# eragonruan/text-detection-ctpn

Hardware: NVIDIA H100
Metric: images/sec @600x900 (higher is better)
Workload: dtype fp32-faithful: fp16 operands + e4m3 cross terms (1 fp16 + 1 e4m3 wgmma per 16 MACs: 2 bf16-rate units per MAC), fp32 accumulate; matmuls around the BiLSTM on bf16x2

## Files before the change

### text-detection-ctpn_b200/csrc/conv_tc.cu

```cuda
#include <cuda.h>

#include <algorithm>
#include <mutex>
#include <unordered_map>

#include "common.cuh"
#include "tc_ptx.cuh"
#include "tma_host.cuh"

namespace ctpn {

#ifdef CTPN_DEBUG
#define CTPN_DBG(p, bit) (((p).debug & (bit)) != 0)
#else
#define CTPN_DBG(p, bit) false
#endif

struct ConvTcParams {
  int B, H, W, Cin, Cout, taps, planes, flags;
  int tiles_x, tiles_y, tiles_n, total_tiles;
  int m_tiles, total_units;
  int TH, TW, tw_log2;
  int PW;
  int patch_bytes;
  int patch_tx_bytes;
  int group_stride_bytes;
  int cout_pad;
  int Ho, Wo;
  int stages_a, stages_b;
  int debug;
  const float *bias;
  void *out;
  long long out_plane_stride;
  float inv_main, inv_cross, out_s, out_t, out_rs;
  int in_stack_h, out_rows, out_stacked;
  const int *ext;
  int ext_shift, ext_n;
  double work;
  int stage_small;
  int promote_every;
};

constexpr int kTcThreads = 384;
constexpr int kMaxStages = 8;
constexpr int kCtrlBytes = 8 * (4 * kMaxStages) + 16;
constexpr int kStagePitch = 64;
constexpr int kEpiBytes = 2 * 128 * 32 * 4;

template <int BN, int P, int TAPS, int MC, int F8, int PR = 0>
__global__ void __launch_bounds__(kTcThreads, 1)
conv_tc_kernel(const __grid_constant__ CUtensorMap tmap_a, const __grid_constant__ CUtensorMap tmap_b,
               const ConvTcParams p) {
  using namespace ptx;
  constexpr int kBBytes = BN * 128;
  static_assert(!F8 || P == 2, "F16F8 uses two stage slots per operand");
  static_assert(!PR || (P == 3 && !F8), "promotion is built for three bf16 planes");
  extern __shared__ uint8_t smem_raw[];
  const uint32_t raw = smem_u32(smem_raw);
  const uint32_t ring_a = (raw + 1023u) & ~1023u;
  const uint32_t a_stage = (uint32_t)P * p.patch_bytes, b_stage = (uint32_t)P * kBBytes;
  const uint32_t ring_b = ring_a + (uint32_t)p.stages_a * a_stage;
  float *epi = reinterpret_cast<float *>(smem_raw + (ring_b - raw) + (size_t)p.stages_b * b_stage);
  uint8_t *ctrl = reinterpret_cast<uint8_t *>(epi) + kEpiBytes;
  const uint32_t fullA = smem_u32(ctrl), emptyA = fullA + 8 * kMaxStages;
  const uint32_t fullB = emptyA + 8 * kMaxStages, emptyB = fullB + 8 * kMaxStages;

  const int warp = __shfl_sync(0xffffffffu, (int)(threadIdx.x >> 5), 0), lane = threadIdx.x & 31;
  if (threadIdx.x == 0) {
    prefetch_tmap(&tmap_a);
    prefetch_tmap(&tmap_b);
    for (int s = 0; s < kMaxStages; ++s) {
      mbar_init(fullA + 8 * s, 1);
      mbar_init(emptyA + 8 * s, 2);
      mbar_init(fullB + 8 * s, 1);
      mbar_init(emptyB + 8 * s, MC ? 4 : 2);
    }
    fence_mbar_init();
  }
  __syncthreads();
  if (MC) cluster_sync_all();
  const uint32_t rank = MC ? cluster_ctarank() : 0u;
  const int u_begin = MC ? (int)(blockIdx.x >> 1) : (int)blockIdx.x, u_step = MC ? (int)(gridDim.x >> 1) : (int)gridDim.x;
  auto unit_tile = [&](int u, int &mt, int &nt) {
    nt = u % p.tiles_n;
    mt = u / p.tiles_n;
    if (MC) mt = min(2 * mt + (int)rank, p.m_tiles - 1);
  };

  const int kblocks = p.Cin / 64;
  const int tiles_per_img = p.tiles_x * p.tiles_y;
  constexpr int halo = TAPS == 9 ? 1 : 0;

  if (warp < 4) {
    regs_dealloc<40>();
    if (warp == 1) {
      int s = 0;
      uint32_t ph = 0;
      for (int u = u_begin; u < p.total_units; u += u_step) {
        int mt, nt;
        unit_tile(u, mt, nt);
        const int b = mt / tiles_per_img, r = mt % tiles_per_img;
        const int y0 = (r / p.tiles_x) * p.TH - halo, x0 = (r % p.tiles_x) * p.TW - halo;
        for (int kb = 0; kb < kblocks; ++kb) {
          mbar_wait(emptyA + 8 * s, ph ^ 1u);
          if (elect_one()) {
            if (CTPN_DBG(p, 2)) { mbar_arrive(fullA + 8 * s); }
            else {
              mbar_arrive_expect_tx(fullA + 8 * s, (uint32_t)P * (uint32_t)p.patch_tx_bytes);
              for (int pl = 0; pl < P; ++pl)
                tma_load_4d(&tmap_a, fullA + 8 * s, ring_a + s * a_stage + pl * p.patch_bytes, kb * 64, x0, y0, pl * p.B + b);
            }
          }
          __syncwarp();
          if (++s == p.stages_a) { s = 0; ph ^= 1u; }
        }
      }
    } else if (warp == 0) {
      int s = 0;
      uint32_t ph = 0;
      for (int u = u_begin; u < p.total_units; u += u_step) {
        int mt, nt;
        unit_tile(u, mt, nt);
        for (int kb = 0; kb < kblocks; ++kb) {
          for (int tap = 0; tap < TAPS; ++tap) {
            mbar_wait(emptyB + 8 * s, ph ^ 1u);
            if (elect_one()) {
              if (CTPN_DBG(p, 1)) { mbar_arrive(fullB + 8 * s); }
              else {
                mbar_arrive_expect_tx(fullB + 8 * s, b_stage);
                for (int pl = 0; pl < P; ++pl) {
                  if (MC)
                    tma_load_2d_mc(&tmap_b, fullB + 8 * s, ring_b + s * b_stage + pl * kBBytes + rank * (kBBytes / 2),
                                   tap * p.Cin + kb * 64, pl * p.cout_pad + nt * BN + (int)rank * (BN / 2), (uint16_t)3);
                  else
                    tma_load_2d(&tmap_b, fullB + 8 * s, ring_b + s * b_stage + pl * kBBytes, tap * p.Cin + kb * 64,
                                pl * p.cout_pad + nt * BN);
                }
              }
            }
            __syncwarp();
            if (++s == p.stages_b) { s = 0; ph ^= 1u; }
          }
        }
      }
    }
  } else {
    regs_alloc<232>();
    const int wg = (warp >> 2) - 1;
    const bool leader = (threadIdx.x & 127) == 0;
    constexpr int R = BN / 2;
    float accm[R], accc[R];
    float accs[R];
#ifdef CTPN_DEBUG
    const int pe = PR ? p.promote_every : 1;
#else
    constexpr int pe = 1;
#endif
    constexpr uint32_t kPatch16 = (TAPS == 9 ? 23552u : 16384u) >> 4;
    constexpr uint32_t kB16 = (uint32_t)kBBytes >> 4;
    constexpr uint32_t kHiB = gmma_desc_hi(1024);
    const uint32_t hi_a = gmma_desc_hi((uint32_t)p.group_stride_bytes);
    const uint32_t wg_off = (uint32_t)wg * 8u * (uint32_t)p.group_stride_bytes;
    const int cw = warp - 4, eset = cw >> 2, quarter = cw & 3;
    const int m = quarter * 32 + lane;
    const int th = m >> p.tw_log2, tw = m & (p.TW - 1);
    const bool pool = (p.flags & CTPN_F_POOL) != 0, relu = (p.flags & CTPN_F_RELU) != 0;
    const bool out_f32 = (p.flags & CTPN_F_OUT_F32) != 0;
    int sa = 0, sb = 0, prev_b = -1, prev_a = -1;
    uint32_t pha = 0, phb = 0;
    auto release = [&](int sbx, int sax) {
      if (leader) {
        if (MC) {
          mbar_arrive_cluster(emptyB + 8 * sbx, 0u);
          mbar_arrive_cluster(emptyB + 8 * sbx, 1u);
        } else {
          mbar_arrive(emptyB + 8 * sbx);
        }
        if (sax >= 0) mbar_arrive(emptyA + 8 * sax);
      }
    };
    for (int u = u_begin; u < p.total_units; u += u_step) {
      if (PR) {
#pragma unroll
        for (int i = 0; i < R; ++i) accs[i] = 0.f;
      }
      for (int kb = 0; kb < kblocks; ++kb) {
        if (p.stages_a == 1 && prev_a >= 0) {
          wgmma_wait<0>();
          release(prev_b, prev_a);
          prev_b = prev_a = -1;
        }
        mbar_wait(fullA + 8 * sa, pha);
        const uint32_t a_lo = gmma_desc_lo(ring_a + sa * a_stage + wg_off);
#pragma unroll
        for (int tap = 0; tap < TAPS; ++tap) {
          mbar_wait(fullB + 8 * sb, phb);
          const uint32_t b_lo = gmma_desc_lo(ring_b + sb * b_stage);
          constexpr int kPW = 10;
          const uint32_t view16 = TAPS == 9 ? (uint32_t)((tap / 3) * kPW + tap % 3) * 8u : 0u;
          const uint32_t not_first = (kb | tap) != 0;
          const int step = kb * TAPS + tap;
          wgmma_fence();
          if (!CTPN_DBG(p, 4)) {
            if (F8) {
#pragma unroll
              for (int k = 0; k < 4; ++k)
                wgmma_f16(accm, ((uint64_t)hi_a << 32) | (a_lo + view16 + 2u * k), ((uint64_t)kHiB << 32) | (b_lo + 2u * k),
                          k == 0 ? not_first : 1u);
#pragma unroll
              for (int k = 0; k < 4; ++k)
                wgmma_e4m3(accc, ((uint64_t)hi_a << 32) | (a_lo + kPatch16 + view16 + 2u * k),
                           ((uint64_t)kHiB << 32) | (b_lo + kB16 + 2u * k), k == 0 ? not_first : 1u);
            } else if (PR) {
              const uint32_t chain_on = step % pe != 0;
#pragma unroll
              for (int k = 0; k < 4; ++k)
                wgmma_bf16(accm, ((uint64_t)hi_a << 32) | (a_lo + view16 + 2u * k), ((uint64_t)kHiB << 32) | (b_lo + 2u * k),
                           k == 0 ? chain_on : 1u);
              wgmma_commit();
#pragma unroll
              for (int i = 0; i < P; ++i) {
#pragma unroll
                for (int j = (i == 0); j < P - i; ++j) {
#pragma unroll
                  for (int k = 0; k < 4; ++k) {
                    const uint64_t da = ((uint64_t)hi_a << 32) | (a_lo + i * kPatch16 + view16 + 2u * k);
                    const uint64_t db = ((uint64_t)kHiB << 32) | (b_lo + j * kB16 + 2u * k);
                    wgmma_bf16(accc, da, db, (k == 0 && i == 0 && j == 1) ? not_first : 1u);
                  }
                }
              }
            } else {
#pragma unroll
              for (int i = 0; i < P; ++i) {
#pragma unroll
                for (int j = 0; j < P - i; ++j) {
#pragma unroll
                  for (int k = 0; k < 4; ++k) {
                    const uint64_t da = ((uint64_t)hi_a << 32) | (a_lo + i * kPatch16 + view16 + 2u * k);
                    const uint64_t db = ((uint64_t)kHiB << 32) | (b_lo + j * kB16 + 2u * k);
                    if (i + j == 0) wgmma_bf16(accm, da, db, k == 0 ? not_first : 1u);
                    else wgmma_bf16(accc, da, db, (k == 0 && i == 0 && j == 1) ? not_first : 1u);
                  }
                }
              }
            }
          }
          wgmma_commit();
          wgmma_wait<1>();
          if (prev_b >= 0) release(prev_b, prev_a);
          prev_b = sb;
          prev_a = tap == TAPS - 1 ? sa : -1;
          if (PR && ((step + 1) % pe == 0 || step == kblocks * TAPS - 1)) {
            wgmma_fence_regs(accm);
#pragma unroll
            for (int i = 0; i < R; ++i) accs[i] = __fadd_rn(accs[i], accm[i]);
          }
          if (++sb == p.stages_b) { sb = 0; phb ^= 1u; }
        }
        if (++sa == p.stages_a) { sa = 0; pha ^= 1u; }
      }
      wgmma_wait<0>();
      wgmma_fence_regs(accm);
      if (P > 1) wgmma_fence_regs(accc);
      if (prev_b >= 0) release(prev_b, prev_a);
      prev_b = prev_a = -1;
      if (P > 1) {
#pragma unroll
        for (int i = 0; i < R; ++i)
          accm[i] = F8 ? __fmaf_rn(accc[i], p.inv_cross, accm[i] * p.inv_main) : PR ? __fadd_rn(accs[i], accc[i]) : accm[i] + accc[i];
      }

      int mt, nt;
      unit_tile(u, mt, nt);
      const int b = mt / tiles_per_img, r = mt % tiles_per_img;
      const int y = (r / p.tiles_x) * p.TH + th, x = (r % p.tiles_x) * p.TW + tw;
      bool ok, live = true;
      int oy, ox, ob = b;
      if (pool) {
        oy = y >> 1; ox = x >> 1;
        ok = !(th & 1) && !(tw & 1) && oy < p.Ho && ox < p.Wo;
      } else {
        oy = y; ox = x;
        ok = y < p.H && x < p.W;
        if (p.in_stack_h) {
          ob = y / p.in_stack_h;
          oy = y - ob * p.in_stack_h;
          live = oy < p.in_stack_h - 1;
          if (!p.out_stacked) ok = ok && live;
        }
      }
      if (p.ext) {
        const int ib = min(ob, p.ext_n - 1);
        live = live && oy < (__ldg(p.ext + 2 * ib) >> p.ext_shift) && ox < (__ldg(p.ext + 2 * ib + 1) >> p.ext_shift);
      }
      const long long pix = ((long long)ob * p.out_rows + oy) * p.Wo + ox;
      const unsigned okmask = __ballot_sync(0xffffffffu, ok);
      long long spix[4];
#pragma unroll
      for (int it = 0; it < 4; ++it) {
        const long long hi = __shfl_sync(0xffffffffu, (int)(pix >> 32), it * 8 + (lane >> 2));
        const unsigned lo = __shfl_sync(0xffffffffu, (unsigned)(pix & 0xffffffffll), it * 8 + (lane >> 2));
        spix[it] = (hi << 32) | lo;
      }
      uint4 *stage_w = reinterpret_cast<uint4 *>(epi + eset * 4096 + quarter * 1024);
      const int frow = wg * 64 + (warp & 3) * 16 + (lane >> 2);
      if (!CTPN_DBG(p, 16)) {
#pragma unroll
      for (int c2 = 0; c2 < BN / 64; ++c2) {
        named_sync(1, 256);
#pragma unroll
        for (int j = 0; j < 8; ++j) {
          const int i8 = c2 * 8 + j, q = 2 * (j & 3) + ((lane & 3) >> 1);
#pragma unroll
          for (int h = 0; h < 2; ++h) {
            const int row = frow + 8 * h;
            *reinterpret_cast<float2 *>(epi + (j >> 2) * 4096 + row * 32 + ((q ^ (row & 7)) << 2) + 2 * (lane & 1)) =
                make_float2(accm[4 * i8 + 2 * h], accm[4 * i8 + 2 * h + 1]);
          }
        }
        named_sync(1, 256);
        const int chunk = 2 * c2 + eset;
        const int c0 = nt * BN + chunk * 32;
        float v[32];
#pragma unroll
        for (int q = 0; q < 8; ++q) {
          const float4 t = *reinterpret_cast<const float4 *>(epi + eset * 4096 + m * 32 + ((q ^ (m & 7)) << 2));
          v[4 * q + 0] = t.x; v[4 * q + 1] = t.y; v[4 * q + 2] = t.z; v[4 * q + 3] = t.w;
        }
#pragma unroll
        for (int q = 0; q < 8; ++q) {
          const float4 bq = __ldg(reinterpret_cast<const float4 *>(p.bias + c0) + q);
          v[4 * q + 0] += bq.x;
          v[4 * q + 1] += bq.y;
          v[4 * q + 2] += bq.z;
          v[4 * q + 3] += bq.w;
        }
        if (relu) {
#pragma unroll
          for (int i = 0; i < 32; ++i) v[i] = fmaxf(v[i], 0.f);
        }
        if (!live) {
#pragma unroll
          for (int i = 0; i < 32; ++i) v[i] = 0.f;
        }
        if (pool) {
#pragma unroll
          for (int i = 0; i < 32; ++i) {
            v[i] = fmaxf(v[i], __shfl_xor_sync(0xffffffffu, v[i], 1));
            v[i] = fmaxf(v[i], __shfl_xor_sync(0xffffffffu, v[i], p.TW));
          }
        }
        if (F8 && pool && !out_f32 && !(p.flags & CTPN_F_OUT_BF16X2)) {
          const int j = (lane & 1) | ((lane >> 2) & 2);
          float x[8];
#pragma unroll
          for (int k = 0; k < 8; ++k) x[k] = j == 0 ? v[k] : j == 1 ? v[8 + k] : j == 2 ? v[16 + k] : v[24 + k];
          const bool okw = oy < p.Ho && ox < p.Wo;
          uint4 hw;
          uint2 qv, qr;
          f16f8_quad(x[0], x[1], x[2], x[3], p.out_s, p.out_t, p.out_rs, hw.x, hw.y, qv.x, qr.x);
          f16f8_quad(x[4], x[5], x[6], x[7], p.out_s, p.out_t, p.out_rs, hw.z, hw.w, qv.y, qr.y);
          if (okw && c0 < p.Cout && !CTPN_DBG(p, 8)) {
            uint8_t *o0 = reinterpret_cast<uint8_t *>(p.out) + pix * p.Cout * 2;
            uint8_t *o1 = o0 + p.out_plane_stride * 2 + (long long)(c0 >> 6) * 128 + (c0 & 63) + j * 8;
            *reinterpret_cast<uint4 *>(o0 + (long long)c0 * 2 + j * 16) = hw;
            *reinterpret_cast<uint2 *>(o1) = qv;
            *reinterpret_cast<uint2 *>(o1 + 64) = qr;
          }
        } else if (F8 && !out_f32 && !(p.flags & CTPN_F_OUT_BF16X2)) {
          uint32_t wh[16], wq[16];
#pragma unroll
          for (int i = 0; i < 8; ++i) {
            f16f8_quad(v[4 * i], v[4 * i + 1], v[4 * i + 2], v[4 * i + 3], p.out_s, p.out_t, p.out_rs, wh[2 * i], wh[2 * i + 1], wq[i], wq[8 + i]);
          }
          const int j = lane & 3;
#pragma unroll
          for (int pl = 0; pl < 2; ++pl) {
            uint8_t *obase = reinterpret_cast<uint8_t *>(p.out) + (long long)pl * p.out_plane_stride * 2;
            const long long off = pl == 0 ? (long long)c0 * 2 + j * 16
                                          : (long long)(c0 >> 6) * 128 + (c0 & 63) + (j >> 1) * 64 + (j & 1) * 16;
            const bool st_ok = c0 < p.Cout && !CTPN_DBG(p, 8);
            if (!p.stage_small) {
              __syncwarp();
#pragma unroll
              for (int q = 0; q < 4; ++q) {
                const uint4 val = pl == 0 ? make_uint4(wh[4 * q], wh[4 * q + 1], wh[4 * q + 2], wh[4 * q + 3])
                                          : make_uint4(wq[4 * q], wq[4 * q + 1], wq[4 * q + 2], wq[4 * q + 3]);
                stage_w[lane * 4 + (q ^ ((lane >> 1) & 3))] = val;
              }
              __syncwarp();
              if (st_ok) {
#pragma unroll
                for (int it = 0; it < 4; ++it) {
                  const int pp = it * 8 + (lane >> 2);
                  const uint4 val = stage_w[pp * 4 + (j ^ ((pp >> 1) & 3))];
                  if ((okmask >> pp) & 1u) *reinterpret_cast<uint4 *>(obase + spix[it] * p.Cout * 2 + off) = val;
                }
              }
            } else {
#pragma unroll
              for (int it = 0; it < 4; ++it) {
                __syncwarp();
                if ((lane >> 3) == it) {
                  const int row = lane & 7;
#pragma unroll
                  for (int q = 0; q < 4; ++q) {
                    const uint4 val = pl == 0 ? make_uint4(wh[4 * q], wh[4 * q + 1], wh[4 * q + 2], wh[4 * q + 3])
                                              : make_uint4(wq[4 * q], wq[4 * q + 1], wq[4 * q + 2], wq[4 * q + 3]);
                    stage_w[row * 4 + (q ^ ((row >> 1) & 3))] = val;
                  }
                }
                __syncwarp();
                const int row = lane >> 2, pp = it * 8 + row;
                const uint4 val = stage_w[row * 4 + (j ^ ((row >> 1) & 3))];
                if (st_ok && ((okmask >> pp) & 1u)) *reinterpret_cast<uint4 *>(obase + spix[it] * p.Cout * 2 + off) = val;
              }
            }
          }
        } else if (!out_f32) {
          uint32_t w[P][16];
#pragma unroll
          for (int i = 0; i < 16; ++i) {
            uint32_t t[P];
            split_planes2<P>(v[2 * i], v[2 * i + 1], t);
#pragma unroll
            for (int pl = 0; pl < P; ++pl) w[pl][i] = t[pl];
          }
#pragma unroll
          for (int pl = 0; pl < P; ++pl) {
            __syncwarp();
#pragma unroll
            for (int q = 0; q < 4; ++q) stage_w[lane * 4 + (q ^ ((lane >> 1) & 3))] = make_uint4(w[pl][4 * q], w[pl][4 * q + 1], w[pl][4 * q + 2], w[pl][4 * q + 3]);
            __syncwarp();
            if (c0 < p.Cout && !CTPN_DBG(p, 8)) {
              __nv_bfloat16 *obase = reinterpret_cast<__nv_bfloat16 *>(p.out) + (long long)pl * p.out_plane_stride + c0 + (lane & 3) * 8;
#pragma unroll
              for (int it = 0; it < 4; ++it) {
                const int pp = it * 8 + (lane >> 2);
                const uint4 val = stage_w[pp * 4 + ((lane & 3) ^ ((pp >> 1) & 3))];
                if ((okmask >> pp) & 1u) *reinterpret_cast<uint4 *>(obase + spix[it] * p.Cout) = val;
              }
            }
          }
        } else if (ok && c0 < p.Cout && !CTPN_DBG(p, 8)) {
          if (out_f32) {
            float4 *dst = reinterpret_cast<float4 *>(reinterpret_cast<float *>(p.out) + pix * p.Cout + c0);
#pragma unroll
            for (int q = 0; q < 8; ++q) dst[q] = make_float4(v[4 * q], v[4 * q + 1], v[4 * q + 2], v[4 * q + 3]);
          }
        }
      }
      }
    }
  }
  __syncthreads();
  if (MC) cluster_sync_all();
}


constexpr int kMaxDevices = 64;
static std::mutex g_mu;
static int g_sms[kMaxDevices];

struct Tuning { int debug = 0, bn = 0, stages_a = 0, stages_b = 0, mcast = 1, stage_small = 1, promote = 1; };
static const Tuning &tuning() {
  static const Tuning t = [] {
    Tuning v;
#ifdef CTPN_DEBUG
    auto env_int = [](const char *name, int dflt) { const char *e = getenv(name); return e ? atoi(e) : dflt; };
    v.debug = env_int("CTPN_TC_DEBUG", 0);
    v.bn = env_int("CTPN_TC_BN", 0);
    v.stages_a = env_int("CTPN_TC_STAGES_A", 0);
    v.stages_b = env_int("CTPN_TC_STAGES_B", 0);
    v.mcast = env_int("CTPN_TC_MCAST", 1);
    v.stage_small = env_int("CTPN_TC_STAGE_SMALL", 1);
    v.promote = std::max(1, env_int("CTPN_TC_PROMOTE", 1));
#endif
    return v;
  }();
  return t;
}

struct TmapKey {
  const void *ptr;
  unsigned long long d0, d1, d2, d3;
  unsigned b0, b1, b2, b3;
  int dev;
  bool operator==(const TmapKey &o) const {
    return ptr == o.ptr && d0 == o.d0 && d1 == o.d1 && d2 == o.d2 && d3 == o.d3 && b0 == o.b0 && b1 == o.b1 && b2 == o.b2 &&
           b3 == o.b3 && dev == o.dev;
  }
};
struct TmapKeyHash {
  size_t operator()(const TmapKey &k) const {
    size_t h = std::hash<const void *>()(k.ptr);
    for (unsigned long long v : {k.d0, k.d1, k.d2, k.d3, (unsigned long long)k.b0, (unsigned long long)k.b1,
                                 (unsigned long long)k.b2, (unsigned long long)k.b3, (unsigned long long)k.dev})
      h = h * 1000003u ^ std::hash<unsigned long long>()(v);
    return h;
  }
};
static std::unordered_map<TmapKey, CUtensorMap, TmapKeyHash> g_tmaps;

static int cached_tmap(int dev, CUtensorMap *out, const void *ptr, int rank, const cuuint64_t *dims, const cuuint64_t *strides,
                       const cuuint32_t *box) {
  TmapKey k{ptr, dims[0], dims[1], rank > 2 ? dims[2] : 0, rank > 3 ? dims[3] : 0, box[0], box[1], rank > 2 ? box[2] : 0,
            rank > 3 ? box[3] : 0, dev};
  std::lock_guard<std::mutex> lock(g_mu);
  auto it = g_tmaps.find(k);
  if (it != g_tmaps.end()) { *out = it->second; return CTPN_OK; }
  EncodeTiledFn enc = nullptr;
  int rc = tma_get_encode(&enc);
  if (rc) return rc;
  if ((rc = tma_encode_bf16(enc, out, const_cast<void *>(ptr), rank, dims, strides, box))) return rc;
  if (g_tmaps.size() >= 1024) g_tmaps.clear();
  g_tmaps.emplace(k, *out);
  return CTPN_OK;
}

template <int BN, int P, int TAPS, int MC, int F8 = 0, int PR = 0>
static int launch_bn(int dev, const CUtensorMap &ta, const CUtensorMap &tb, ConvTcParams &p, cudaStream_t st) {
  const size_t a_stage = (size_t)p.planes * p.patch_bytes, b_stage = (size_t)p.planes * BN * 128;
  const bool small = F8 && TAPS == 9 && p.Cin >= 256 && !(p.flags & (CTPN_F_OUT_F32 | CTPN_F_OUT_BF16X2 | CTPN_F_POOL)) && tuning().stage_small != 0;
  p.stage_small = small ? 1 : 0;
  const size_t budget = 227 * 1024 - 1024 - kCtrlBytes - kEpiBytes;
  int sa = (2 * a_stage + 2 * b_stage <= budget) ? 2 : 1;
  if (p.taps == 1) sa = (int)std::min<size_t>(4, std::max<size_t>(1, (budget / 2) / a_stage));
  CTPN_REQUIRE(sa * a_stage + 2 * b_stage <= budget, "conv_tc: pipeline stages (%zu + 2 x %zu B) do not fit in shared memory", a_stage, b_stage);
  int sb = (int)((budget - sa * a_stage) / b_stage);
  if (sb > kMaxStages) sb = kMaxStages;
  if (tuning().stages_a > 0) sa = std::max(1, std::min(sa, tuning().stages_a));
  if (tuning().stages_b > 0) sb = std::max(2, std::min(sb, tuning().stages_b));
  p.stages_a = sa;
  p.stages_b = sb;
  const size_t smem = 1024 + sa * a_stage + sb * b_stage + kEpiBytes + kCtrlBytes;
  CTPN_REQUIRE(smem <= 227 * 1024, "conv_tc: %zu bytes of shared memory", smem);
  auto kernel = conv_tc_kernel<BN, P, TAPS, MC, F8, PR>;
  static bool attr_set[kMaxDevices];
  static int max_clusters[kMaxDevices];
  cudaLaunchConfig_t cfg = {};
  cudaLaunchAttribute attr;
  attr.id = cudaLaunchAttributeClusterDimension;
  attr.val.clusterDim.x = 2; attr.val.clusterDim.y = 1; attr.val.clusterDim.z = 1;
  cfg.blockDim = dim3(kTcThreads);
  cfg.dynamicSmemBytes = smem;
  cfg.stream = st;
  cfg.attrs = &attr;
  cfg.numAttrs = MC ? 1 : 0;
  {
    std::lock_guard<std::mutex> lock(g_mu);
    if (!attr_set[dev]) {
      CTPN_CUDA(cudaFuncSetAttribute(kernel, cudaFuncAttributeMaxDynamicSharedMemorySize, 227 * 1024));
      if (MC) {
        cfg.gridDim = dim3(2 * (g_sms[dev] / 2));
        int n = 0;
        CTPN_CUDA(cudaOccupancyMaxActiveClusters(&n, kernel, &cfg));
        CTPN_REQUIRE(n > 0, "conv_tc: no 2-CTA cluster of this kernel fits on the device");
        max_clusters[dev] = n;
      }
      attr_set[dev] = true;
    }
  }
  char label[128];
  if (prof_enabled()) snprintf(label, sizeof(label), "conv_tc t%d %dx%dx%d c%d-%d %s%d bn%d%s%s", p.taps, p.B, p.H, p.W, p.Cin, p.Cout, F8 ? "f16f8 p" : "p", p.planes, BN, MC ? " mc" : "", PR ? " promote" : "");
  ProfScope prof(label, p.work, st);
  if (MC) cfg.gridDim = dim3(2 * std::min(max_clusters[dev], p.total_units));
  else cfg.gridDim = dim3(std::min(p.total_units, g_sms[dev]));
  CTPN_CUDA(cudaLaunchKernelEx(&cfg, kernel, ta, tb, p));
  CTPN_LAUNCH_CHECK();
  return CTPN_OK;
}

int conv_tc_run(const void *in_planes, const void *w_planes, const float *bias, void *out, int B, int H, int W, int cin,
                int cout, int taps, int planes, int flags, const QuantScales *q, const int *ext, int ext_shift, void *stream) {
  const bool f8 = q != nullptr, promote = (flags & CTPN_F_PROMOTE) != 0;
  CTPN_REQUIRE(f8 || !(flags & CTPN_F_OUT_BF16X2), "ctpn_conv3x3: CTPN_F_OUT_BF16X2 is a flag of ctpn_conv3x3_f16f8");
  CTPN_REQUIRE(!(promote && f8), "ctpn_conv3x3_f16f8: CTPN_F_PROMOTE is a flag of ctpn_conv3x3 with planes = 3");
  CTPN_REQUIRE(!promote || planes == 3, "ctpn_conv3x3: CTPN_F_PROMOTE needs planes = 3 (got %d)", planes);
  CTPN_REQUIRE(in_planes && w_planes && bias && out, "ctpn_conv3x3: null pointer");
  CTPN_REQUIRE(taps == 9 || taps == 1, "ctpn_conv3x3: taps must be 9 or 1 (got %d)", taps);
  CTPN_REQUIRE(planes >= 1 && planes <= 3, "ctpn_conv3x3: planes must be 1..3 (got %d)", planes);
  CTPN_REQUIRE(cin % 64 == 0 && cin >= 64, "ctpn_conv3x3: Cin must be a multiple of 64 (got %d)", cin);
  CTPN_REQUIRE(cout % 64 == 0 && cout >= 64, "ctpn_conv3x3: Cout must be a multiple of 64 (got %d)", cout);
  CTPN_REQUIRE(B > 0 && H > 0 && W > 0, "ctpn_conv3x3: bad shape");
  const bool pool = flags & CTPN_F_POOL;
  CTPN_REQUIRE(!pool || (taps == 9 && H >= 2 && W >= 2), "ctpn_conv3x3: pooling needs taps=9 and H,W >= 2");
  const bool stack_in = flags & CTPN_F_STACK_IN, stack_out = flags & CTPN_F_STACK_OUT;
  CTPN_REQUIRE(!stack_in || (taps == 9 && !pool), "ctpn_conv3x3: CTPN_F_STACK_IN needs taps=9 and no pooling");
  CTPN_REQUIRE(!stack_out || !(flags & CTPN_F_OUT_F32), "ctpn_conv3x3: stacked output is a plane format");
  const int img_B = B, img_H = H;
  if (stack_in) {
    CTPN_REQUIRE((long long)B * (H + 1) < (1ll << 30), "ctpn_conv3x3: stack too tall");
    H = B * (H + 1);
    B = 1;
  }
  int dev = 0, rc;
  CTPN_CUDA(cudaGetDevice(&dev));
  CTPN_REQUIRE(dev >= 0 && dev < kMaxDevices, "ctpn_conv3x3: device index %d not supported", dev);
  {
    std::lock_guard<std::mutex> lock(g_mu);
    if (g_sms[dev] == 0) CTPN_CUDA(cudaDeviceGetAttribute(&g_sms[dev], cudaDevAttrMultiProcessorCount, dev));
  }

  ConvTcParams p;
  memset(&p, 0, sizeof(p));
  p.B = B; p.H = H; p.W = W; p.Cin = cin; p.Cout = cout; p.taps = taps; p.planes = planes; p.flags = flags;
  if (taps == 9) {
    p.TH = 16; p.TW = 8; p.tw_log2 = 3;
    p.PW = 10;
    p.group_stride_bytes = p.PW * 128;
    p.patch_tx_bytes = p.PW * 18 * 128;
    p.patch_bytes = (int)align_up((size_t)p.patch_tx_bytes, 1024);
  } else {
    p.TH = 1; p.TW = 128; p.tw_log2 = 7;
    p.PW = 128;
    p.group_stride_bytes = 1024;
    p.patch_tx_bytes = 128 * 128;
    p.patch_bytes = 128 * 128;
  }
  p.tiles_x = ceil_div(W, p.TW);
  p.tiles_y = ceil_div(H, p.TH);
  p.Ho = pool ? H / 2 : H;
  p.Wo = pool ? W / 2 : W;
  p.bias = bias;
  p.out = out;
  p.work = 2.0 * img_B * img_H * W * (double)taps * cin * cout;
  p.in_stack_h = stack_in ? img_H + 1 : 0;
  const int img_Ho = pool ? img_H / 2 : img_H;
  p.out_rows = img_Ho + (stack_out ? 1 : 0);
  p.out_stacked = stack_out ? 1 : 0;
  p.out_plane_stride = (long long)img_B * p.out_rows * p.Wo * cout;
  p.cout_pad = cout;
  p.ext = ext;
  p.ext_shift = ext_shift;
  p.ext_n = img_B;
  if (f8) {
    CTPN_REQUIRE(q->inv_main > 0.f && q->inv_cross > 0.f && q->out_s > 0.f && q->out_t > 0.f, "ctpn_conv3x3_f16f8: scales must be positive");
    p.inv_main = q->inv_main; p.inv_cross = q->inv_cross; p.out_s = q->out_s; p.out_t = q->out_t;
    p.out_rs = kResidualGain * q->out_t / q->out_s;
  }
  p.debug = tuning().debug;
  p.promote_every = tuning().promote;

  int BN = tuning().bn > 0 ? tuning().bn : (planes == 1 ? 256 : 128);
  if (!(BN == 64 || BN == 128 || BN == 256)) BN = 256;
  if (planes > 1 && BN > 128) BN = 128;
  while (BN > cout || cout % BN) BN >>= 1;
  const long long m_tiles = (long long)B * p.tiles_x * p.tiles_y;
  constexpr long long kMcMaxTilesPerSm = 16;
  const bool mc = taps == 9 && tuning().mcast != 0 && m_tiles >= 2 &&
                  (promote || m_tiles * (cout / BN) < kMcMaxTilesPerSm * g_sms[dev]);
  if (promote && taps == 9 && !mc && BN > 64) BN = 64;
  p.tiles_n = cout / BN;
  const long long total = m_tiles * p.tiles_n;
  CTPN_REQUIRE(total < (1ll << 31), "ctpn_conv3x3: too many tiles");
  p.total_tiles = (int)total;
  p.m_tiles = (int)m_tiles;
  p.total_units = mc ? (int)((m_tiles + 1) / 2) * p.tiles_n : p.total_tiles;

  CUtensorMap ta, tb;
  {
    const int halo = taps == 9 ? 1 : 0;
    cuuint64_t dims[4] = {(cuuint64_t)cin, (cuuint64_t)W, (cuuint64_t)H, (cuuint64_t)planes * B};
    cuuint64_t strides[3] = {(cuuint64_t)cin * 2, (cuuint64_t)W * cin * 2, (cuuint64_t)H * W * cin * 2};
    cuuint32_t box[4] = {64, (cuuint32_t)p.PW, (cuuint32_t)(p.TH + 2 * halo), 1};
    if ((rc = cached_tmap(dev, &ta, in_planes, 4, dims, strides, box))) return rc;
  }
  {
    cuuint64_t dims[2] = {(cuuint64_t)taps * cin, (cuuint64_t)planes * cout};
    cuuint64_t strides[1] = {(cuuint64_t)taps * cin * 2};
    cuuint32_t box[2] = {64, (cuuint32_t)(mc ? BN / 2 : BN)};
    if ((rc = cached_tmap(dev, &tb, w_planes, 2, dims, strides, box))) return rc;
  }
  cudaStream_t st = (cudaStream_t)stream;
#define CTPN_TC_CASE(BN_, P_, T_) \
  if (BN == BN_ && planes == P_ && taps == T_) return launch_bn<BN_, P_, T_, 0>(dev, ta, tb, p, st)
#define CTPN_TC_CASE_MC(BN_, P_) \
  if (mc && BN == BN_ && planes == P_) return launch_bn<BN_, P_, 9, 1>(dev, ta, tb, p, st)
  if (f8) {
    if (mc && BN == 128) return launch_bn<128, 2, 9, 1, 1>(dev, ta, tb, p, st);
    if (mc && BN == 64) return launch_bn<64, 2, 9, 1, 1>(dev, ta, tb, p, st);
    if (taps == 9 && BN == 128) return launch_bn<128, 2, 9, 0, 1>(dev, ta, tb, p, st);
    if (taps == 9 && BN == 64) return launch_bn<64, 2, 9, 0, 1>(dev, ta, tb, p, st);
    if (taps == 1 && BN == 128) return launch_bn<128, 2, 1, 0, 1>(dev, ta, tb, p, st);
    if (taps == 1 && BN == 64) return launch_bn<64, 2, 1, 0, 1>(dev, ta, tb, p, st);
    set_error("ctpn_conv3x3_f16f8: no kernel for BN=%d taps=%d", BN, taps);
    return CTPN_ERR_INVALID;
  }
  if (promote) {
    if (mc && BN == 128) return launch_bn<128, 3, 9, 1, 0, 1>(dev, ta, tb, p, st);
    if (mc && BN == 64) return launch_bn<64, 3, 9, 1, 0, 1>(dev, ta, tb, p, st);
    if (taps == 9 && BN == 64) return launch_bn<64, 3, 9, 0, 0, 1>(dev, ta, tb, p, st);
    if (taps == 1 && BN == 128) return launch_bn<128, 3, 1, 0, 0, 1>(dev, ta, tb, p, st);
    if (taps == 1 && BN == 64) return launch_bn<64, 3, 1, 0, 0, 1>(dev, ta, tb, p, st);
    set_error("ctpn_conv3x3: no promoted kernel for BN=%d taps=%d", BN, taps);
    return CTPN_ERR_INVALID;
  }
  CTPN_TC_CASE_MC(256, 1); CTPN_TC_CASE_MC(128, 1); CTPN_TC_CASE_MC(64, 1);
  CTPN_TC_CASE_MC(128, 2); CTPN_TC_CASE_MC(64, 2);
  CTPN_TC_CASE_MC(128, 3); CTPN_TC_CASE_MC(64, 3);
  CTPN_TC_CASE(256, 1, 9); CTPN_TC_CASE(128, 1, 9); CTPN_TC_CASE(64, 1, 9);
  CTPN_TC_CASE(128, 2, 9); CTPN_TC_CASE(64, 2, 9);
  CTPN_TC_CASE(128, 3, 9); CTPN_TC_CASE(64, 3, 9);
  CTPN_TC_CASE(256, 1, 1); CTPN_TC_CASE(128, 1, 1); CTPN_TC_CASE(64, 1, 1);
  CTPN_TC_CASE(128, 2, 1); CTPN_TC_CASE(64, 2, 1);
  CTPN_TC_CASE(128, 3, 1); CTPN_TC_CASE(64, 3, 1);
#undef CTPN_TC_CASE_MC
#undef CTPN_TC_CASE
  set_error("ctpn_conv3x3: no kernel for BN=%d planes=%d taps=%d", BN, planes, taps);
  return CTPN_ERR_INVALID;
}

}

using namespace ctpn;

extern "C" int ctpn_conv3x3(const void *in_planes, const void *w_planes, const float *bias, void *out, int B, int H,
                            int W, int cin, int cout, int taps, int planes, int flags, void *stream) {
  return conv_tc_run(in_planes, w_planes, bias, out, B, H, W, cin, cout, taps, planes, flags, nullptr, nullptr, 0, stream);
}

extern "C" int ctpn_conv3x3_f16f8(const void *in_planes, const void *w_planes, const float *bias, void *out, int B, int H,
                                  int W, int cin, int cout, int taps, int flags, float inv_main, float inv_cross, float out_s,
                                  float out_t, void *stream) {
  const QuantScales q{inv_main, inv_cross, out_s, out_t};
  return conv_tc_run(in_planes, w_planes, bias, out, B, H, W, cin, cout, taps, 2, flags, &q, nullptr, 0, stream);
}
```

Measured before the change: 762.7.

## Offload conv epilogue to idle producer warps to overlap with next tile's MMA

Adds an epilogue-warp variant where warps 2-3 of the producer group take over bias, ReLU, pooling, quantisation and stores. The consumer warpgroups only dump accumulators to shared memory and then move on to the next tile's wgmma. For wide tiles, chunks beyond the two in the epilogue buffer are staged in the last A pipeline slot, whose release is deferred until the epilogue warps finish. This drops the register dealloc/alloc split, so the MMA warpgroups no longer get the larger 232-register allocation. It also adds mbarrier hand-off latency and can stall the producer on the A slot.

```diff
diff --git a/text-detection-ctpn_b200/csrc/conv_tc.cu b/text-detection-ctpn_b200/csrc/conv_tc.cu
--- a/text-detection-ctpn_b200/csrc/conv_tc.cu
+++ b/text-detection-ctpn_b200/csrc/conv_tc.cu
@@ -46,8 +46,200 @@
 constexpr int kCtrlBytes = 8 * (4 * kMaxStages) + 16;
 constexpr int kStagePitch = 64;
 constexpr int kEpiBytes = 2 * 128 * 32 * 4;
-
-template <int BN, int P, int TAPS, int MC, int F8, int PR = 0>
+constexpr int kChunkFloats = 128 * 32;
+
+__device__ __forceinline__ float *stage_at(float *chunk, int row, int i8, int lane) {
+  const int q = 2 * (i8 & 3) + ((lane & 3) >> 1);
+  return chunk + row * 32 + ((q ^ (row & 7)) << 2) + 2 * (lane & 1);
+}
+
+struct EpiPixel {
+  long long pix;
+  long long spix[4];
+  unsigned okmask;
+  int oy, ox;
+  bool ok, live;
+};
+
+__device__ __forceinline__ EpiPixel epi_pixel(const ConvTcParams &p, int mt, int m, int lane) {
+  EpiPixel e;
+  const int tiles_per_img = p.tiles_x * p.tiles_y;
+  const int th = m >> p.tw_log2, tw = m & (p.TW - 1);
+  const int b = mt / tiles_per_img, r = mt % tiles_per_img;
+  const int y = (r / p.tiles_x) * p.TH + th, x = (r % p.tiles_x) * p.TW + tw;
+  int ob = b;
+  e.live = true;
+  if (p.flags & CTPN_F_POOL) {
+    e.oy = y >> 1; e.ox = x >> 1;
+    e.ok = !(th & 1) && !(tw & 1) && e.oy < p.Ho && e.ox < p.Wo;
+  } else {
+    e.oy = y; e.ox = x;
+    e.ok = y < p.H && x < p.W;
+    if (p.in_stack_h) {
+      ob = y / p.in_stack_h;
+      e.oy = y - ob * p.in_stack_h;
+      e.live = e.oy < p.in_stack_h - 1;
+      if (!p.out_stacked) e.ok = e.ok && e.live;
+    }
+  }
+  if (p.ext) {
+    const int ib = min(ob, p.ext_n - 1);
+    e.live = e.live && e.oy < (__ldg(p.ext + 2 * ib) >> p.ext_shift) && e.ox < (__ldg(p.ext + 2 * ib + 1) >> p.ext_shift);
+  }
+  e.pix = ((long long)ob * p.out_rows + e.oy) * p.Wo + e.ox;
+  e.okmask = __ballot_sync(0xffffffffu, e.ok);
+#pragma unroll
+  for (int it = 0; it < 4; ++it) {
+    const long long hi = __shfl_sync(0xffffffffu, (int)(e.pix >> 32), it * 8 + (lane >> 2));
+    const unsigned lo = __shfl_sync(0xffffffffu, (unsigned)(e.pix & 0xffffffffll), it * 8 + (lane >> 2));
+    e.spix[it] = (hi << 32) | lo;
+  }
+  return e;
+}
+
+template <int P, int F8>
+__device__ __forceinline__ void epi_chunk(const ConvTcParams &p, float *chunk, int m, int lane, int c0, const EpiPixel &e) {
+  const bool pool = (p.flags & CTPN_F_POOL) != 0, relu = (p.flags & CTPN_F_RELU) != 0;
+  const bool out_f32 = (p.flags & CTPN_F_OUT_F32) != 0;
+  const long long pix = e.pix;
+  const int oy = e.oy, ox = e.ox;
+  uint4 *stage_w = reinterpret_cast<uint4 *>(chunk + (m & ~31) * 32);
+  float v[32];
+#pragma unroll
+  for (int q = 0; q < 8; ++q) {
+    const float4 t = *reinterpret_cast<const float4 *>(chunk + m * 32 + ((q ^ (m & 7)) << 2));
+    v[4 * q + 0] = t.x; v[4 * q + 1] = t.y; v[4 * q + 2] = t.z; v[4 * q + 3] = t.w;
+  }
+#pragma unroll
+  for (int q = 0; q < 8; ++q) {
+    const float4 bq = __ldg(reinterpret_cast<const float4 *>(p.bias + c0) + q);
+    v[4 * q + 0] += bq.x;
+    v[4 * q + 1] += bq.y;
+    v[4 * q + 2] += bq.z;
+    v[4 * q + 3] += bq.w;
+  }
+  if (relu) {
+#pragma unroll
+    for (int i = 0; i < 32; ++i) v[i] = fmaxf(v[i], 0.f);
+  }
+  if (!e.live) {
+#pragma unroll
+    for (int i = 0; i < 32; ++i) v[i] = 0.f;
+  }
+  if (pool) {
+#pragma unroll
+    for (int i = 0; i < 32; ++i) {
+      v[i] = fmaxf(v[i], __shfl_xor_sync(0xffffffffu, v[i], 1));
+      v[i] = fmaxf(v[i], __shfl_xor_sync(0xffffffffu, v[i], p.TW));
+    }
+  }
+  if (F8 && pool && !out_f32 && !(p.flags & CTPN_F_OUT_BF16X2)) {
+    const int j = (lane & 1) | ((lane >> 2) & 2);
+    float x[8];
+#pragma unroll
+    for (int k = 0; k < 8; ++k) x[k] = j == 0 ? v[k] : j == 1 ? v[8 + k] : j == 2 ? v[16 + k] : v[24 + k];
+    const bool okw = oy < p.Ho && ox < p.Wo;
+    uint4 hw;
+    uint2 qv, qr;
+    f16f8_quad(x[0], x[1], x[2], x[3], p.out_s, p.out_t, p.out_rs, hw.x, hw.y, qv.x, qr.x);
+    f16f8_quad(x[4], x[5], x[6], x[7], p.out_s, p.out_t, p.out_rs, hw.z, hw.w, qv.y, qr.y);
+    if (okw && c0 < p.Cout && !CTPN_DBG(p, 8)) {
+      uint8_t *o0 = reinterpret_cast<uint8_t *>(p.out) + pix * p.Cout * 2;
+      uint8_t *o1 = o0 + p.out_plane_stride * 2 + (long long)(c0 >> 6) * 128 + (c0 & 63) + j * 8;
+      *reinterpret_cast<uint4 *>(o0 + (long long)c0 * 2 + j * 16) = hw;
+      *reinterpret_cast<uint2 *>(o1) = qv;
+      *reinterpret_cast<uint2 *>(o1 + 64) = qr;
+    }
+  } else if (F8 && !out_f32 && !(p.flags & CTPN_F_OUT_BF16X2)) {
+    uint32_t wh[16], wq[16];
+#pragma unroll
+    for (int i = 0; i < 8; ++i) {
+      f16f8_quad(v[4 * i], v[4 * i + 1], v[4 * i + 2], v[4 * i + 3], p.out_s, p.out_t, p.out_rs, wh[2 * i], wh[2 * i + 1], wq[i], wq[8 + i]);
+    }
+    const int j = lane & 3;
+#pragma unroll
+    for (int pl = 0; pl < 2; ++pl) {
+      uint8_t *obase = reinterpret_cast<uint8_t *>(p.out) + (long long)pl * p.out_plane_stride * 2;
+      const long long off = pl == 0 ? (long long)c0 * 2 + j * 16
+                                    : (long long)(c0 >> 6) * 128 + (c0 & 63) + (j >> 1) * 64 + (j & 1) * 16;
+      const bool st_ok = c0 < p.Cout && !CTPN_DBG(p, 8);
+      if (!p.stage_small) {
+        __syncwarp();
+#pragma unroll
+        for (int q = 0; q < 4; ++q) {
+          const uint4 val = pl == 0 ? make_uint4(wh[4 * q], wh[4 * q + 1], wh[4 * q + 2], wh[4 * q + 3])
+                                    : make_uint4(wq[4 * q], wq[4 * q + 1], wq[4 * q + 2], wq[4 * q + 3]);
+          stage_w[lane * 4 + (q ^ ((lane >> 1) & 3))] = val;
+        }
+        __syncwarp();
+        if (st_ok) {
+#pragma unroll
+          for (int it = 0; it < 4; ++it) {
+            const int pp = it * 8 + (lane >> 2);
+            const uint4 val = stage_w[pp * 4 + (j ^ ((pp >> 1) & 3))];
+            if ((e.okmask >> pp) & 1u) *reinterpret_cast<uint4 *>(obase + e.spix[it] * p.Cout * 2 + off) = val;
+          }
+        }
+      } else {
+#pragma unroll
+        for (int it = 0; it < 4; ++it) {
+          __syncwarp();
+          if ((lane >> 3) == it) {
+            const int row = lane & 7;
+#pragma unroll
+            for (int q = 0; q < 4; ++q) {
+              const uint4 val = pl == 0 ? make_uint4(wh[4 * q], wh[4 * q + 1], wh[4 * q + 2], wh[4 * q + 3])
+                                        : make_uint4(wq[4 * q], wq[4 * q + 1], wq[4 * q + 2], wq[4 * q + 3]);
+              stage_w[row * 4 + (q ^ ((row >> 1) & 3))] = val;
+            }
+          }
+          __syncwarp();
+          const int row = lane >> 2, pp = it * 8 + row;
+          const uint4 val = stage_w[row * 4 + (j ^ ((row >> 1) & 3))];
+          if (st_ok && ((e.okmask >> pp) & 1u)) *reinterpret_cast<uint4 *>(obase + e.spix[it] * p.Cout * 2 + off) = val;
+        }
+      }
+    }
+  } else if (!out_f32) {
+    uint32_t w[P][16];
+#pragma unroll
+    for (int i = 0; i < 16; ++i) {
+      uint32_t t[P];
+      split_planes2<P>(v[2 * i], v[2 * i + 1], t);
+#pragma unroll
+      for (int pl = 0; pl < P; ++pl) w[pl][i] = t[pl];
+    }
+#pragma unroll
+    for (int pl = 0; pl < P; ++pl) {
+      __syncwarp();
+#pragma unroll
+      for (int q = 0; q < 4; ++q) stage_w[lane * 4 + (q ^ ((lane >> 1) & 3))] = make_uint4(w[pl][4 * q], w[pl][4 * q + 1], w[pl][4 * q + 2], w[pl][4 * q + 3]);
+      __syncwarp();
+      if (c0 < p.Cout && !CTPN_DBG(p, 8)) {
+        __nv_bfloat16 *obase = reinterpret_cast<__nv_bfloat16 *>(p.out) + (long long)pl * p.out_plane_stride + c0 + (lane & 3) * 8;
+#pragma unroll
+        for (int it = 0; it < 4; ++it) {
+          const int pp = it * 8 + (lane >> 2);
+          const uint4 val = stage_w[pp * 4 + ((lane & 3) ^ ((pp >> 1) & 3))];
+          if ((e.okmask >> pp) & 1u) *reinterpret_cast<uint4 *>(obase + e.spix[it] * p.Cout) = val;
+        }
+      }
+    }
+  } else if (e.ok && c0 < p.Cout && !CTPN_DBG(p, 8)) {
+    if (out_f32) {
+      float4 *dst = reinterpret_cast<float4 *>(reinterpret_cast<float *>(p.out) + pix * p.Cout + c0);
+#pragma unroll
+      for (int q = 0; q < 8; ++q) dst[q] = make_float4(v[4 * q], v[4 * q + 1], v[4 * q + 2], v[4 * q + 3]);
+    }
+  }
+}
+
+template <int BN, int P, int TAPS, int PR>
+__host__ __device__ constexpr bool epi_warps_fit() {
+  return !PR && (BN / 32 - 2) * kChunkFloats * 4 <= P * (TAPS == 9 ? 23552 : 16384);
+}
+
+template <int BN, int P, int TAPS, int MC, int F8, int PR = 0, int EW = 0>
 __global__ void __launch_bounds__(kTcThreads, 1)
 conv_tc_kernel(const __grid_constant__ CUtensorMap tmap_a, const __grid_constant__ CUtensorMap tmap_b,
                const ConvTcParams p) {
@@ -55,6 +247,10 @@
   constexpr int kBBytes = BN * 128;
   static_assert(!F8 || P == 2, "F16F8 uses two stage slots per operand");
   static_assert(!PR || (P == 3 && !F8), "promotion is built for three bf16 planes");
+  constexpr int kChunks = BN / 32;
+  static_assert(!EW || epi_warps_fit<BN, P, TAPS, PR>(), "the tile does not fit the hand-off buffer");
+  constexpr bool kEpiWarps = EW != 0;
+  constexpr bool kHandoffA = kEpiWarps && kChunks > 2;
   extern __shared__ uint8_t smem_raw[];
   const uint32_t raw = smem_u32(smem_raw);
   const uint32_t ring_a = (raw + 1023u) & ~1023u;
@@ -64,6 +260,11 @@
   uint8_t *ctrl = reinterpret_cast<uint8_t *>(epi) + kEpiBytes;
   const uint32_t fullA = smem_u32(ctrl), emptyA = fullA + 8 * kMaxStages;
   const uint32_t fullB = emptyA + 8 * kMaxStages, emptyB = fullB + 8 * kMaxStages;
+  const uint32_t hfull = emptyB + 8 * kMaxStages, hempty = hfull + 8;
+  auto chunk_at = [&](int c, int sa_last) {
+    return c < 2 ? epi + c * kChunkFloats
+                 : reinterpret_cast<float *>(smem_raw + (ring_a - raw) + (size_t)sa_last * a_stage) + (c - 2) * kChunkFloats;
+  };
 
   const int warp = __shfl_sync(0xffffffffu, (int)(threadIdx.x >> 5), 0), lane = threadIdx.x & 31;
   if (threadIdx.x == 0) {
@@ -75,6 +276,8 @@
       mbar_init(fullB + 8 * s, 1);
       mbar_init(emptyB + 8 * s, MC ? 4 : 2);
     }
+    mbar_init(hfull, 2);
+    mbar_init(hempty, 2);
     fence_mbar_init();
   }
   __syncthreads();
@@ -92,7 +295,7 @@
   constexpr int halo = TAPS == 9 ? 1 : 0;
 
   if (warp < 4) {
-    regs_dealloc<40>();
+    if (!kEpiWarps) regs_dealloc<40>();
     if (warp == 1) {
       int s = 0;
       uint32_t ph = 0;
@@ -143,9 +346,41 @@
           }
         }
       }
+    } else if (kEpiWarps) {
+      const int ew = warp - 2;
+      int sa_next = 0;
+      uint32_t ph = 0;
+      for (int u = u_begin; u < p.total_units; u += u_step) {
+        const int sa_last = (sa_next + kblocks - 1) % p.stages_a;
+        sa_next = (sa_next + kblocks) % p.stages_a;
+        int mt, nt;
+        unit_tile(u, mt, nt);
+        mbar_wait(hfull, ph);
+#pragma unroll 1
+        for (int half = kHandoffA ? 0 : 1; half < 2; ++half) {
+          const int c_begin = half == 0 ? 2 : 0, c_end = half == 0 || !kHandoffA ? kChunks : 2;
+          if (!CTPN_DBG(p, 16)) {
+#pragma unroll 1
+            for (int pass = 0; pass < 2; ++pass) {
+              const int m = (2 * pass + ew) * 32 + lane;
+              const EpiPixel e = epi_pixel(p, mt, m, lane);
+#pragma unroll 1
+              for (int c = c_begin; c < c_end; ++c) epi_chunk<P, F8>(p, chunk_at(c, sa_last), m, lane, nt * BN + c * 32, e);
+            }
+          }
+          if (half == 0) {
+            fence_proxy_async();
+            __syncwarp();
+            if (lane == 0) mbar_arrive(emptyA + 8 * sa_last);
+          }
+        }
+        __syncwarp();
+        if (lane == 0) mbar_arrive(hempty);
+        ph ^= 1u;
+      }
     }
   } else {
-    regs_alloc<232>();
+    if (!kEpiWarps) regs_alloc<232>();
     const int wg = (warp >> 2) - 1;
     const bool leader = (threadIdx.x & 127) == 0;
     constexpr int R = BN / 2;
@@ -163,11 +398,9 @@
     const uint32_t wg_off = (uint32_t)wg * 8u * (uint32_t)p.group_stride_bytes;
     const int cw = warp - 4, eset = cw >> 2, quarter = cw & 3;
     const int m = quarter * 32 + lane;
-    const int th = m >> p.tw_log2, tw = m & (p.TW - 1);
-    const bool pool = (p.flags & CTPN_F_POOL) != 0, relu = (p.flags & CTPN_F_RELU) != 0;
-    const bool out_f32 = (p.flags & CTPN_F_OUT_F32) != 0;
+    const int frow = wg * 64 + (warp & 3) * 16 + (lane >> 2);
     int sa = 0, sb = 0, prev_b = -1, prev_a = -1;
-    uint32_t pha = 0, phb = 0;
+    uint32_t pha = 0, phb = 0, phe = 0;
     auto release = [&](int sbx, int sax) {
       if (leader) {
         if (MC) {
@@ -263,194 +496,47 @@
       wgmma_wait<0>();
       wgmma_fence_regs(accm);
       if (P > 1) wgmma_fence_regs(accc);
-      if (prev_b >= 0) release(prev_b, prev_a);
+      const int sa_last = prev_a;
+      if (prev_b >= 0) release(prev_b, kHandoffA ? -1 : prev_a);
       prev_b = prev_a = -1;
       if (P > 1) {
 #pragma unroll
         for (int i = 0; i < R; ++i)
           accm[i] = F8 ? __fmaf_rn(accc[i], p.inv_cross, accm[i] * p.inv_main) : PR ? __fadd_rn(accs[i], accc[i]) : accm[i] + accc[i];
       }
+      if (kEpiWarps) {
+        mbar_wait(hempty, phe ^ 1u);
+        phe ^= 1u;
+        if (kHandoffA) named_sync(1, 256);
+#pragma unroll
+        for (int i8 = 0; i8 < BN / 8; ++i8) {
+          float *chunk = chunk_at(i8 >> 2, sa_last);
+#pragma unroll
+          for (int h = 0; h < 2; ++h)
+            *reinterpret_cast<float2 *>(stage_at(chunk, frow + 8 * h, i8, lane)) = make_float2(accm[4 * i8 + 2 * h], accm[4 * i8 + 2 * h + 1]);
+        }
+        named_sync(2 + wg, 128);
+        if (leader) mbar_arrive(hfull);
+        continue;
+      }
 
       int mt, nt;
       unit_tile(u, mt, nt);
-      const int b = mt / tiles_per_img, r = mt % tiles_per_img;
-      const int y = (r / p.tiles_x) * p.TH + th, x = (r % p.tiles_x) * p.TW + tw;
-      bool ok, live = true;
-      int oy, ox, ob = b;
-      if (pool) {
-        oy = y >> 1; ox = x >> 1;
-        ok = !(th & 1) && !(tw & 1) && oy < p.Ho && ox < p.Wo;
-      } else {
-        oy = y; ox = x;
-        ok = y < p.H && x < p.W;
-        if (p.in_stack_h) {
-          ob = y / p.in_stack_h;
-          oy = y - ob * p.in_stack_h;
-          live = oy < p.in_stack_h - 1;
-          if (!p.out_stacked) ok = ok && live;
-        }
-      }
-      if (p.ext) {
-        const int ib = min(ob, p.ext_n - 1);
-        live = live && oy < (__ldg(p.ext + 2 * ib) >> p.ext_shift) && ox < (__ldg(p.ext + 2 * ib + 1) >> p.ext_shift);
-      }
-      const long long pix = ((long long)ob * p.out_rows + oy) * p.Wo + ox;
-      const unsigned okmask = __ballot_sync(0xffffffffu, ok);
-      long long spix[4];
-#pragma unroll
-      for (int it = 0; it < 4; ++it) {
-        const long long hi = __shfl_sync(0xffffffffu, (int)(pix >> 32), it * 8 + (lane >> 2));
-        const unsigned lo = __shfl_sync(0xffffffffu, (unsigned)(pix & 0xffffffffll), it * 8 + (lane >> 2));
-        spix[it] = (hi << 32) | lo;
-      }
-      uint4 *stage_w = reinterpret_cast<uint4 *>(epi + eset * 4096 + quarter * 1024);
-      const int frow = wg * 64 + (warp & 3) * 16 + (lane >> 2);
+      const EpiPixel e = epi_pixel(p, mt, m, lane);
       if (!CTPN_DBG(p, 16)) {
 #pragma unroll
-      for (int c2 = 0; c2 < BN / 64; ++c2) {
-        named_sync(1, 256);
-#pragma unroll
-        for (int j = 0; j < 8; ++j) {
-          const int i8 = c2 * 8 + j, q = 2 * (j & 3) + ((lane & 3) >> 1);
-#pragma unroll
-          for (int h = 0; h < 2; ++h) {
-            const int row = frow + 8 * h;
-            *reinterpret_cast<float2 *>(epi + (j >> 2) * 4096 + row * 32 + ((q ^ (row & 7)) << 2) + 2 * (lane & 1)) =
-                make_float2(accm[4 * i8 + 2 * h], accm[4 * i8 + 2 * h + 1]);
+        for (int c2 = 0; c2 < BN / 64; ++c2) {
+          named_sync(1, 256);
+#pragma unroll
+          for (int j = 0; j < 8; ++j) {
+#pragma unroll
+            for (int h = 0; h < 2; ++h)
+              *reinterpret_cast<float2 *>(stage_at(epi + (j >> 2) * kChunkFloats, frow + 8 * h, j, lane)) =
+                  make_float2(accm[4 * (c2 * 8 + j) + 2 * h], accm[4 * (c2 * 8 + j) + 2 * h + 1]);
           }
-        }
-        named_sync(1, 256);
-        const int chunk = 2 * c2 + eset;
-        const int c0 = nt * BN + chunk * 32;
-        float v[32];
-#pragma unroll
-        for (int q = 0; q < 8; ++q) {
-          const float4 t = *reinterpret_cast<const float4 *>(epi + eset * 4096 + m * 32 + ((q ^ (m & 7)) << 2));
-          v[4 * q + 0] = t.x; v[4 * q + 1] = t.y; v[4 * q + 2] = t.z; v[4 * q + 3] = t.w;
-        }
-#pragma unroll
-        for (int q = 0; q < 8; ++q) {
-          const float4 bq = __ldg(reinterpret_cast<const float4 *>(p.bias + c0) + q);
-          v[4 * q + 0] += bq.x;
-          v[4 * q + 1] += bq.y;
-          v[4 * q + 2] += bq.z;
-          v[4 * q + 3] += bq.w;
-        }
-        if (relu) {
-#pragma unroll
-          for (int i = 0; i < 32; ++i) v[i] = fmaxf(v[i], 0.f);
-        }
-        if (!live) {
-#pragma unroll
-          for (int i = 0; i < 32; ++i) v[i] = 0.f;
-        }
-        if (pool) {
-#pragma unroll
-          for (int i = 0; i < 32; ++i) {
-            v[i] = fmaxf(v[i], __shfl_xor_sync(0xffffffffu, v[i], 1));
-            v[i] = fmaxf(v[i], __shfl_xor_sync(0xffffffffu, v[i], p.TW));
-          }
-        }
-        if (F8 && pool && !out_f32 && !(p.flags & CTPN_F_OUT_BF16X2)) {
-          const int j = (lane & 1) | ((lane >> 2) & 2);
-          float x[8];
-#pragma unroll
-          for (int k = 0; k < 8; ++k) x[k] = j == 0 ? v[k] : j == 1 ? v[8 + k] : j == 2 ? v[16 + k] : v[24 + k];
-          const bool okw = oy < p.Ho && ox < p.Wo;
-          uint4 hw;
-          uint2 qv, qr;
-          f16f8_quad(x[0], x[1], x[2], x[3], p.out_s, p.out_t, p.out_rs, hw.x, hw.y, qv.x, qr.x);
-          f16f8_quad(x[4], x[5], x[6], x[7], p.out_s, p.out_t, p.out_rs, hw.z, hw.w, qv.y, qr.y);
-          if (okw && c0 < p.Cout && !CTPN_DBG(p, 8)) {
-            uint8_t *o0 = reinterpret_cast<uint8_t *>(p.out) + pix * p.Cout * 2;
-            uint8_t *o1 = o0 + p.out_plane_stride * 2 + (long long)(c0 >> 6) * 128 + (c0 & 63) + j * 8;
-            *reinterpret_cast<uint4 *>(o0 + (long long)c0 * 2 + j * 16) = hw;
-            *reinterpret_cast<uint2 *>(o1) = qv;
-            *reinterpret_cast<uint2 *>(o1 + 64) = qr;
-          }
-        } else if (F8 && !out_f32 && !(p.flags & CTPN_F_OUT_BF16X2)) {
-          uint32_t wh[16], wq[16];
-#pragma unroll
-          for (int i = 0; i < 8; ++i) {
-            f16f8_quad(v[4 * i], v[4 * i + 1], v[4 * i + 2], v[4 * i + 3], p.out_s, p.out_t, p.out_rs, wh[2 * i], wh[2 * i + 1], wq[i], wq[8 + i]);
-          }
-          const int j = lane & 3;
-#pragma unroll
-          for (int pl = 0; pl < 2; ++pl) {
-            uint8_t *obase = reinterpret_cast<uint8_t *>(p.out) + (long long)pl * p.out_plane_stride * 2;
-            const long long off = pl == 0 ? (long long)c0 * 2 + j * 16
-                                          : (long long)(c0 >> 6) * 128 + (c0 & 63) + (j >> 1) * 64 + (j & 1) * 16;
-            const bool st_ok = c0 < p.Cout && !CTPN_DBG(p, 8);
-            if (!p.stage_small) {
-              __syncwarp();
-#pragma unroll
-              for (int q = 0; q < 4; ++q) {
-                const uint4 val = pl == 0 ? make_uint4(wh[4 * q], wh[4 * q + 1], wh[4 * q + 2], wh[4 * q + 3])
-                                          : make_uint4(wq[4 * q], wq[4 * q + 1], wq[4 * q + 2], wq[4 * q + 3]);
-                stage_w[lane * 4 + (q ^ ((lane >> 1) & 3))] = val;
-              }
-              __syncwarp();
-              if (st_ok) {
-#pragma unroll
-                for (int it = 0; it < 4; ++it) {
-                  const int pp = it * 8 + (lane >> 2);
-                  const uint4 val = stage_w[pp * 4 + (j ^ ((pp >> 1) & 3))];
-                  if ((okmask >> pp) & 1u) *reinterpret_cast<uint4 *>(obase + spix[it] * p.Cout * 2 + off) = val;
-                }
-              }
-            } else {
-#pragma unroll
-              for (int it = 0; it < 4; ++it) {
-                __syncwarp();
-                if ((lane >> 3) == it) {
-                  const int row = lane & 7;
-#pragma unroll
-                  for (int q = 0; q < 4; ++q) {
-                    const uint4 val = pl == 0 ? make_uint4(wh[4 * q], wh[4 * q + 1], wh[4 * q + 2], wh[4 * q + 3])
-                                              : make_uint4(wq[4 * q], wq[4 * q + 1], wq[4 * q + 2], wq[4 * q + 3]);
-                    stage_w[row * 4 + (q ^ ((row >> 1) & 3))] = val;
-                  }
-                }
-                __syncwarp();
-                const int row = lane >> 2, pp = it * 8 + row;
-                const uint4 val = stage_w[row * 4 + (j ^ ((row >> 1) & 3))];
-                if (st_ok && ((okmask >> pp) & 1u)) *reinterpret_cast<uint4 *>(obase + spix[it] * p.Cout * 2 + off) = val;
-              }
-            }
-          }
-        } else if (!out_f32) {
-          uint32_t w[P][16];
-#pragma unroll
-          for (int i = 0; i < 16; ++i) {
-            uint32_t t[P];
-            split_planes2<P>(v[2 * i], v[2 * i + 1], t);
-#pragma unroll
-            for (int pl = 0; pl < P; ++pl) w[pl][i] = t[pl];
-          }
-#pragma unroll
-          for (int pl = 0; pl < P; ++pl) {
-            __syncwarp();
-#pragma unroll
-            for (int q = 0; q < 4; ++q) stage_w[lane * 4 + (q ^ ((lane >> 1) & 3))] = make_uint4(w[pl][4 * q], w[pl][4 * q + 1], w[pl][4 * q + 2], w[pl][4 * q + 3]);
-            __syncwarp();
-            if (c0 < p.Cout && !CTPN_DBG(p, 8)) {
-              __nv_bfloat16 *obase = reinterpret_cast<__nv_bfloat16 *>(p.out) + (long long)pl * p.out_plane_stride + c0 + (lane & 3) * 8;
-#pragma unroll
-              for (int it = 0; it < 4; ++it) {
-                const int pp = it * 8 + (lane >> 2);
-                const uint4 val = stage_w[pp * 4 + ((lane & 3) ^ ((pp >> 1) & 3))];
-                if ((okmask >> pp) & 1u) *reinterpret_cast<uint4 *>(obase + spix[it] * p.Cout) = val;
-              }
-            }
-          }
-        } else if (ok && c0 < p.Cout && !CTPN_DBG(p, 8)) {
-          if (out_f32) {
-            float4 *dst = reinterpret_cast<float4 *>(reinterpret_cast<float *>(p.out) + pix * p.Cout + c0);
-#pragma unroll
-            for (int q = 0; q < 8; ++q) dst[q] = make_float4(v[4 * q], v[4 * q + 1], v[4 * q + 2], v[4 * q + 3]);
-          }
-        }
-      }
+          named_sync(1, 256);
+          epi_chunk<P, F8>(p, epi + eset * kChunkFloats, m, lane, nt * BN + (2 * c2 + eset) * 32, e);
+        }
       }
     }
   }
@@ -536,9 +622,11 @@
   p.stages_b = sb;
   const size_t smem = 1024 + sa * a_stage + sb * b_stage + kEpiBytes + kCtrlBytes;
   CTPN_REQUIRE(smem <= 227 * 1024, "conv_tc: %zu bytes of shared memory", smem);
-  auto kernel = conv_tc_kernel<BN, P, TAPS, MC, F8, PR>;
-  static bool attr_set[kMaxDevices];
-  static int max_clusters[kMaxDevices];
+  const int ew = epi_warps_fit<BN, P, TAPS, PR>() && p.Cin >= 128 ? 1 : 0;
+  auto kernel = ew ? conv_tc_kernel<BN, P, TAPS, MC, F8, PR, epi_warps_fit<BN, P, TAPS, PR>() ? 1 : 0>
+                   : conv_tc_kernel<BN, P, TAPS, MC, F8, PR, 0>;
+  static bool attr_set[kMaxDevices][2];
+  static int max_clusters[kMaxDevices][2];
   cudaLaunchConfig_t cfg = {};
   cudaLaunchAttribute attr;
   attr.id = cudaLaunchAttributeClusterDimension;
@@ -550,22 +638,22 @@
   cfg.numAttrs = MC ? 1 : 0;
   {
     std::lock_guard<std::mutex> lock(g_mu);
-    if (!attr_set[dev]) {
+    if (!attr_set[dev][ew]) {
       CTPN_CUDA(cudaFuncSetAttribute(kernel, cudaFuncAttributeMaxDynamicSharedMemorySize, 227 * 1024));
       if (MC) {
         cfg.gridDim = dim3(2 * (g_sms[dev] / 2));
         int n = 0;
         CTPN_CUDA(cudaOccupancyMaxActiveClusters(&n, kernel, &cfg));
         CTPN_REQUIRE(n > 0, "conv_tc: no 2-CTA cluster of this kernel fits on the device");
-        max_clusters[dev] = n;
-      }
-      attr_set[dev] = true;
+        max_clusters[dev][ew] = n;
+      }
+      attr_set[dev][ew] = true;
     }
   }
   char label[128];
   if (prof_enabled()) snprintf(label, sizeof(label), "conv_tc t%d %dx%dx%d c%d-%d %s%d bn%d%s%s", p.taps, p.B, p.H, p.W, p.Cin, p.Cout, F8 ? "f16f8 p" : "p", p.planes, BN, MC ? " mc" : "", PR ? " promote" : "");
   ProfScope prof(label, p.work, st);
-  if (MC) cfg.gridDim = dim3(2 * std::min(max_clusters[dev], p.total_units));
+  if (MC) cfg.gridDim = dim3(2 * std::min(max_clusters[dev][ew], p.total_units));
   else cfg.gridDim = dim3(std::min(p.total_units, g_sms[dev]));
   CTPN_CUDA(cudaLaunchKernelEx(&cfg, kernel, ta, tb, p));
   CTPN_LAUNCH_CHECK();
```

Result: faster. 775.3 (median of 6 runs) (+1.7%).
